# CliMA/OrthogonalSphericalShellGrids.jl

Measured on AMD Instinct MI355X. Metric: grid-cells/s metric precompute + zipper halo-fill GB/s, 1/10°×75z, higher is better.
Workload: dtype f64

## Files before the change

### orthogonalsphericalshellgrids.jl_amd/csrc/tpg_batch.hpp

```cpp
#pragma once
#include "tpg_math.hpp"

namespace tpgb {
using namespace tpgm;

#define TPG_UNROLL _Pragma("unroll")

template <int N> TPG_DEV double kc(double c)
{
#if defined(__HIP_DEVICE_COMPILE__)
    if (N == 1) asm("" : "+s"(c));
#endif
    return c;
}

template <int N> TPG_DEV void ksin_b(const double (&x)[N], const double (&y)[N], double (&out)[N])
{
    double z[N], r[N], v[N];
    TPG_UNROLL for (int e = 0; e < N; ++e) z[e] = x[e] * x[e];
    TPG_UNROLL for (int e = 0; e < N; ++e) r[e] = fmaD(z[e], kc<N>(1.58969099521155010221e-10), kc<N>(-2.50507602534068634195e-08));
    TPG_UNROLL for (int e = 0; e < N; ++e) r[e] = fmaD(z[e], r[e], kc<N>(2.75573137070700676789e-06));
    TPG_UNROLL for (int e = 0; e < N; ++e) r[e] = fmaD(z[e], r[e], kc<N>(-1.98412698298579493134e-04));
    TPG_UNROLL for (int e = 0; e < N; ++e) r[e] = fmaD(z[e], r[e], kc<N>(8.33333333332248946124e-03));
    TPG_UNROLL for (int e = 0; e < N; ++e) v[e] = z[e] * x[e];
// ... 8 lines not shown
    TPG_UNROLL for (int e = 0; e < N; ++e) r[e] = fmaD(z[e], r[e], kc<N>(-2.75573143513906633035e-07));
    TPG_UNROLL for (int e = 0; e < N; ++e) r[e] = fmaD(z[e], r[e], kc<N>(2.48015872894767294178e-05));
    TPG_UNROLL for (int e = 0; e < N; ++e) r[e] = fmaD(z[e], r[e], kc<N>(-1.38888888888741095749e-03));
    TPG_UNROLL for (int e = 0; e < N; ++e) r[e] = fmaD(z[e], r[e], kc<N>(4.16666666666666019037e-02));
    TPG_UNROLL for (int e = 0; e < N; ++e) r[e] = z[e] * r[e];
    TPG_UNROLL for (int e = 0; e < N; ++e) {
        double hz = 0.5 * z[e];
        double w = 1.0 - hz;
        out[e] = w + (((1.0 - w) - hz) + (z[e] * r[e] - x[e] * y[e]));
    }
}

template <int N> TPG_DEV void ksin0_b(const double (&x)[N], double (&out)[N])
{
    double z[N], r[N], v[N];
    TPG_UNROLL for (int e = 0; e < N; ++e) z[e] = x[e] * x[e];
    TPG_UNROLL for (int e = 0; e < N; ++e) r[e] = fmaD(z[e], kc<N>(1.58969099521155010221e-10), kc<N>(-2.50507602534068634195e-08));
    TPG_UNROLL for (int e = 0; e < N; ++e) r[e] = fmaD(z[e], r[e], kc<N>(2.75573137070700676789e-06));
    TPG_UNROLL for (int e = 0; e < N; ++e) r[e] = fmaD(z[e], r[e], kc<N>(-1.98412698298579493134e-04));
    TPG_UNROLL for (int e = 0; e < N; ++e) r[e] = fmaD(z[e], r[e], kc<N>(8.33333333332248946124e-03));
    TPG_UNROLL for (int e = 0; e < N; ++e) v[e] = z[e] * x[e];
    TPG_UNROLL for (int e = 0; e < N; ++e) {
        const double t = v[e] * r[e];
        out[e] = x[e] - (z[e] * -t - v[e] * kc<N>(-1.66666666666666324348e-01));
    }
}

template <int N> TPG_DEV bool sin_small_b(const double (&x)[N], double (&out)[N])
{
    bool rare = false;
    TPG_UNROLL for (int e = 0; e < N; ++e) rare |= !(absD(x[e]) <= kPio4Hi);
    ksin0_b<N>(x, out);
    return rare;
}

template <int N> TPG_DEV bool cos_b(const double (&a)[N], double (&out)[N])
{
    double fn[N], y0[N], y1[N], S[N], C[N];
    bool rare = false;
    TPG_UNROLL for (int e = 0; e < N; ++e) fn[e] = __builtin_rint(a[e] * kInvPio2);
    TPG_UNROLL for (int e = 0; e < N; ++e) {
        double r = a[e] - fn[e] * kPio2_1;
        double w = fn[e] * kPio2_1t;
        y0[e] = r - w;
        y1[e] = (r - y0[e]) - w;
        rare |= absD(y0[e]) < absD(a[e]) * 0x1p-15;
    }
    bool odd = false, even = false;
    TPG_UNROLL for (int e = 0; e < N; ++e) { const int n = (int)fn[e]; odd |= (n & 1) != 0; even |= (n & 1) == 0; }
    TPG_UNROLL for (int e = 0; e < N; ++e) { S[e] = 0.0; C[e] = 0.0; }
    if (__any(odd)) ksin_b<N>(y0, y1, S);
    if (__any(even)) kcos_b<N>(y0, y1, C);
    TPG_UNROLL for (int e = 0; e < N; ++e) {
        const int n = (int)fn[e];
        const double v = (n & 1) ? S[e] : C[e];
        const double nv = -v;
        out[e] = ((n + 1) & 2) ? nv : v;
    }
    return rare;
}

template <int N> TPG_DEV bool cos_lat_b(const double (&a)[N], double (&out)[N])
{
    double fn[N], y0[N], y1[N], S[N], C[N];
    bool rare = false;
    TPG_UNROLL for (int e = 0; e < N; ++e) fn[e] = __builtin_rint(a[e] * kInvPio2);
// ... 36 lines not shown
        num = b1 ? n1 : num; den = b1 ? d1 : den; h = b1 ? h1 : h; l = b1 ? l1 : l;
        num = b0 ? n0 : num; den = b0 ? d0 : den; h = b0 ? h0 : h; l = b0 ? l0 : l;
        hi[e] = h; lo[e] = l;
        double q = num / den;
        asm volatile("" : "+v"(q));
        t[e] = direct[e] ? ax : q;
    }
    {
        double z[N], w[N], s1[N], s2[N];
        TPG_UNROLL for (int e = 0; e < N; ++e) { z[e] = t[e] * t[e]; w[e] = z[e] * z[e]; }
        TPG_UNROLL for (int e = 0; e < N; ++e) { s1[e] = fmaD(w[e], 1.62858201153657823623e-02, 4.97687799461593236017e-02);
                                                 s2[e] = fmaD(w[e], -3.65315727442169155270e-02, -5.83357013379057348645e-02); }
        TPG_UNROLL for (int e = 0; e < N; ++e) { s1[e] = fmaD(w[e], s1[e], 6.66107313738753120669e-02);
                                                 s2[e] = fmaD(w[e], s2[e], -7.69187620504482999495e-02); }
        TPG_UNROLL for (int e = 0; e < N; ++e) { s1[e] = fmaD(w[e], s1[e], 9.09088713343650656196e-02);
                                                 s2[e] = fmaD(w[e], s2[e], -1.11111104054623557880e-01); }
        TPG_UNROLL for (int e = 0; e < N; ++e) { s1[e] = fmaD(w[e], s1[e], 1.42857142725034663711e-01);
                                                 s2[e] = fmaD(w[e], s2[e], -1.99999999998764832476e-01); }
        TPG_UNROLL for (int e = 0; e < N; ++e) { s1[e] = fmaD(w[e], s1[e], 3.33333333333329318027e-01);
                                                 s2[e] = w[e] * s2[e]; }
        TPG_UNROLL for (int e = 0; e < N; ++e) s[e] = z[e] * s1[e] + s2[e];
    }
    TPG_UNROLL for (int e = 0; e < N; ++e) {
        const double ts = t[e] * s[e];
        const double rd = t[e] - ts, rg = hi[e] - ((ts - lo[e]) - t[e]);
        const double r = direct[e] ? rd : rg;
        out[e] = csign(r, x[e]);
    }
}

struct AtanRow { double p, q, r, s, hi, lo; };
#define TPG_ATAN_ROWS_DOUBLES 30
#define TPG_ATAN_TABLE_DOUBLES 42
__device__ const unsigned kAtanLutWords[24] = {
    0x30303000u, 0x30303030u, 0x30303030u, 0x30303030u, 0x30303030u, 0x60606030u, 0x60606060u, 0x60606060u,
    0x60606060u, 0x60606060u, 0x60606060u, 0x90606060u, 0x90909090u, 0x90909090u, 0x90909090u, 0x90909090u,
    0x90909090u, 0x90909090u, 0x90909090u, 0x90909090u, 0xC0C0C0C0u, 0xC0C0C0C0u, 0xC0C0C0C0u, 0xC0C0C0C0u };
TPG_DEV void atan_table_init(double* tab, int tid)
{
    if (tid < 24) reinterpret_cast<unsigned*>(tab + TPG_ATAN_ROWS_DOUBLES)[tid] = kAtanLutWords[tid];
    const double rows[5][6] = {
        { 1.0, 0.0, 1.0, 0.0, 0.0, 0.0 },
        { 2.0, 1.0, 2.0, 1.0, 0x1.dac670561bb4fp-2, 0x1.a2b7f222f65e2p-56 },
        { 1.0, 1.0, 1.0, 1.0, 0x1.921fb54442d18p-1, 0x1.1a62633145c07p-55 },
        { 1.0, 1.5, 1.0, 1.5, 0x1.f730bd281f69bp-1, 0x1.007887af0cbbdp-56 },
        { 0.0, 1.0, 0.0, 1.0, kPio2Hi, kPio2Lo } };
    if (tid < TPG_ATAN_ROWS_DOUBLES) tab[tid] = rows[tid / 6][tid % 6];
}

template <int N, bool FINITE = false> TPG_DEV void atan_tab_b(const double (&x)[N], double (&out)[N], const double* tab)
{
    double t[N], hi[N], lo[N], s[N];
    TPG_UNROLL for (int e = 0; e < N; ++e) {
        const double ax = absD(x[e]);
        int u = (int)__builtin_amdgcn_ubfe((unsigned)__double2hiint(x[e]), 15u, 16u) - 0x7FB7;
        u = u < 0 ? 0 : (u > 80 ? 80 : u);
        const unsigned off = reinterpret_cast<const unsigned char*>(tab + TPG_ATAN_ROWS_DOUBLES)[u];
        const AtanRow row = *reinterpret_cast<const AtanRow*>(reinterpret_cast<const char*>(tab) + off);
        hi[e] = row.hi; lo[e] = row.lo;
        const double axn = (!FINITE && ax > 0x1p1000) ? 0x1p1000 : ax;
        const double num = row.p * axn - row.q;
        const double den = row.r + row.s * axn;
        double q = tpgm::div_nr(num, den);
        asm volatile("" : "+v"(q));
        t[e] = q;
    }
    {
        double z[N], w[N], s1[N], s2[N];
        TPG_UNROLL for (int e = 0; e < N; ++e) { z[e] = t[e] * t[e]; w[e] = z[e] * z[e]; }
        TPG_UNROLL for (int e = 0; e < N; ++e) { s1[e] = fmaD(w[e], 1.62858201153657823623e-02, 4.97687799461593236017e-02);
                                                 s2[e] = fmaD(w[e], -3.65315727442169155270e-02, -5.83357013379057348645e-02); }
        TPG_UNROLL for (int e = 0; e < N; ++e) { s1[e] = fmaD(w[e], s1[e], 6.66107313738753120669e-02);
                                                 s2[e] = fmaD(w[e], s2[e], -7.69187620504482999495e-02); }
        TPG_UNROLL for (int e = 0; e < N; ++e) { s1[e] = fmaD(w[e], s1[e], 9.09088713343650656196e-02);
                                                 s2[e] = fmaD(w[e], s2[e], -1.11111104054623557880e-01); }
        TPG_UNROLL for (int e = 0; e < N; ++e) { s1[e] = fmaD(w[e], s1[e], 1.42857142725034663711e-01);
                                                 s2[e] = fmaD(w[e], s2[e], -1.99999999998764832476e-01); }
        TPG_UNROLL for (int e = 0; e < N; ++e) { s1[e] = fmaD(w[e], s1[e], 3.33333333333329318027e-01);
                                                 s2[e] = w[e] * s2[e]; }
        TPG_UNROLL for (int e = 0; e < N; ++e) s[e] = z[e] * s1[e] + s2[e];
// ... 88 lines not shown
    double h[N], l[N], S[N], C[N];
    bool s1[N], c1[N], rare = false;
    TPG_UNROLL for (int e = 0; e < N; ++e) {
        const double r = absD(x[e]);
        rare |= !(r <= 90.0);
        s1[e] = r >= 45.0; c1[e] = r > 45.0;
        const double d = (s1[e] ? 90.0 : 0.0) - r;
        const double t = absD(d);
        const double hh = t * kDeg2Rad;
        l[e] = fmaD(t, kDeg2Rad, -hh) + t * kDeg2RadLo;
        h[e] = hh;
    }
    ksin_b<N>(h, l, S);
    kcos_b<N>(h, l, C);
    TPG_UNROLL for (int e = 0; e < N; ++e) {
        const double bs = s1[e] ? C[e] : S[e];
        sn[e] = csign(1.0, x[e]) * bs;
        cs[e] = c1[e] ? S[e] : C[e];
    }
    return rare;
}

TPG_DEV double fmod360_pos(double x)
{
    return x - __hiloint2double(!(x < 360.0) ? 0x40768000 : 0, 0);
}

TPG_DEV double fmod360_small(double x)
{
    const double ax = absD(x);
    return csign(ax - __hiloint2double(!(ax < 360.0) ? 0x40768000 : 0, 0), x);
}

}
```

### orthogonalsphericalshellgrids.jl_amd/csrc/tpg_grid.hip

```cpp
#include "tpg_common.hpp"
#include "tpg_math.hpp"
#include "tpg_batch.hpp"

using namespace tpgm;

namespace {

constexpr double kC180Pi = 180.0 / kPi;
constexpr double kC360Pi = 360.0 / kPi;

struct GridK {
    int Nx, Ny, Hx, Hy;
    int shift;
    int jstart, jend;
    int jm_lo, jm_hi;
    int sx, rows;
    int ft;
    double fplp90;
    double R;
    const double* ti;
    const double* tj;
    const double* ts;
};

// ... 162 lines not shown
}
__device__ __forceinline__ double tri_area(V3 a, V3 b, V3 c)
{
    double t = absD(dot3(a, cross3(b, c)));
    t /= 1 + dot3(a, b) + dot3(b, c) + dot3(a, c);
    return 2 * atanD(t);
}
__device__ __forceinline__ double quad_area(V3 a, V3 b, V3 c, V3 d)
{
    double A = tri_area(a, b, c);
    A += tri_area(a, b, d);
    A += tri_area(a, c, d);
    A += tri_area(b, c, d);
    return A / 2;
}

__device__ __forceinline__ double tri_tan_nr(V3 a, V3 b, V3 c)
{
    return div_nr(absD(dot3(a, cross3(b, c))), 1 + dot3(a, b) + dot3(b, c) + dot3(a, c));
}
__device__ __forceinline__ double tri_tan(V3 a, V3 b, V3 c)
{
    return absD(dot3(a, cross3(b, c))) / (1 + dot3(a, b) + dot3(b, c) + dot3(a, c));
}

template <typename T, bool NT = false>
__device__ __forceinline__ void put(const OutPtrs& o, int q, long long off, double v)
{
    T* p = static_cast<T*>(o.p[q]) + off;
    if (NT) __builtin_nontemporal_store((T)v, p); else *p = (T)v;
}

template <typename T, bool NT = false>
__device__ __forceinline__ void put32(const OutPtrs& o, int q, unsigned boff, double v)
{
    asm volatile("" : "+v"(boff));
    T* p = reinterpret_cast<T*>(static_cast<char*>(o.p[q]) + boff);
    if (NT) __builtin_nontemporal_store((T)v, p); else *p = (T)v;
}

template <typename T, bool NT>
__global__ __launch_bounds__(256) void k_cells(GridK g, OutPtrs o)
{
    const int nbx = (g.Nx + 255) / 256;
    int rb = blockIdx.x / nbx;
    int i = (blockIdx.x - rb * nbx) * 256 + threadIdx.x + 1;
    int j = g.jm_lo + rb;
    if (i > g.Nx) return;

    LP cc = coord(g, 0, 0, i, j), fc = coord(g, 1, 0, i, j), cf = coord(g, 0, 1, i, j), ff = coord(g, 1, 1, i, j);
    LP fc_e = coord(g, 1, 0, i + 1, j), fc_s = coord(g, 1, 0, i, j - 1);
    LP cc_w = coord(g, 0, 0, i - 1, j), cc_s = coord(g, 0, 0, i, j - 1), cc_sw = coord(g, 0, 0, i - 1, j - 1);
    LP ff_e = coord(g, 1, 1, i + 1, j), ff_n = coord(g, 1, 1, i, j + 1), ff_ne = coord(g, 1, 1, i + 1, j + 1);
    LP cf_w = coord(g, 0, 1, i - 1, j), cf_n = coord(g, 0, 1, i, j + 1);

    const double R = g.R;
    double dxcc = haversine(fc_e, fc, R);
    double dxfc = haversine(cc, cc_w, R);
    double dxcf = haversine(ff_e, ff, R);
    double dxff = haversine(cf, cf_w, R);
    double dycc = haversine(cf_n, cf, R);
    double dyfc = haversine(ff_n, ff, R);
    double dycf = haversine(cc, cc_s, R);
    double dyff = haversine(fc, fc_s, R);
    double azcc = quad_area(cartesian(ff), cartesian(ff_e), cartesian(ff_ne), cartesian(ff_n)) * (R * R);
    double azfc = dyfc * dxfc;
    double azcf = dycf * dxcf;
    double azff = quad_area(cartesian(cc_sw), cartesian(cc_s), cartesian(cc), cartesian(cc_w)) * (R * R);

    long long off = (long long)(i + g.Hx - 1) + (long long)g.sx * (j - g.jstart + g.Hy);
    put<T, NT>(o, TPG_LAMBDA_CC, off, cc.lam); put<T, NT>(o, TPG_LAMBDA_FC, off, fc.lam);
    put<T, NT>(o, TPG_LAMBDA_CF, off, cf.lam); put<T, NT>(o, TPG_LAMBDA_FF, off, ff.lam);
    put<T, NT>(o, TPG_PHI_CC, off, cc.phi); put<T, NT>(o, TPG_PHI_FC, off, fc.phi);
    put<T, NT>(o, TPG_PHI_CF, off, cf.phi); put<T, NT>(o, TPG_PHI_FF, off, ff.phi);
    put<T, NT>(o, TPG_DX_CC, off, dxcc); put<T, NT>(o, TPG_DX_FC, off, dxfc);
    put<T, NT>(o, TPG_DX_CF, off, dxcf); put<T, NT>(o, TPG_DX_FF, off, dxff);
    put<T, NT>(o, TPG_DY_CC, off, dycc); put<T, NT>(o, TPG_DY_CF, off, dycf);
    put<T, NT>(o, TPG_DY_FC, off, dyfc); put<T, NT>(o, TPG_DY_FF, off, dyff);
    put<T, NT>(o, TPG_AZ_CC, off, azcc); put<T, NT>(o, TPG_AZ_FC, off, azfc);
    put<T, NT>(o, TPG_AZ_CF, off, azcf); put<T, NT>(o, TPG_AZ_FF, off, azff);
}

struct Pt  { double lam, phi, a, ca; };
struct PtX { double lam, phi, a, ca, X, Y, Z; };
struct Nb  { double lam, a, ca; };
struct NbX { double lam, a, ca, X, Y, Z; };

__device__ __forceinline__ Pt make_pt(const GridK& g, int xl, int yl, int i, int j)
{
    LP p = coord(g, xl, yl, i, j);
    Pt r; r.lam = p.lam; r.phi = p.phi; r.a = p.phi * kDeg2Rad; r.ca = cosD(r.a);
    return r;
}
__device__ __forceinline__ PtX make_ptx(const GridK& g, int xl, int yl, int i, int j)
{
    LP p = coord(g, xl, yl, i, j);
    PtX r; r.lam = p.lam; r.phi = p.phi; r.a = p.phi * kDeg2Rad; r.ca = cosD(r.a);
    double sl, cl, sp, cp;
    sincosd(p.lam, sl, cl);
    sincosd(p.phi, sp, cp);
    r.X = cl * cp; r.Y = sl * cp; r.Z = sp;
    return r;
}
__device__ __forceinline__ Nb nb_of(const Pt& p) { return Nb{ p.lam, p.a, p.ca }; }
__device__ __forceinline__ Nb nb_of(const PtX& p) { return Nb{ p.lam, p.a, p.ca }; }
__device__ __forceinline__ NbX nbx_of(const PtX& p) { return NbX{ p.lam, p.a, p.ca, p.X, p.Y, p.Z }; }
__device__ __forceinline__ V3 v3_of(const PtX& p) { return V3{ p.X, p.Y, p.Z }; }
__device__ __forceinline__ V3 v3_of(const NbX& p) { return V3{ p.X, p.Y, p.Z }; }

template <int DIR> __device__ __forceinline__ double shf(double v)
{
    return DIR > 0 ? __shfl_down(v, 1, 64) : __shfl_up(v, 1, 64);
}
template <int DIR> __device__ __forceinline__ Nb shf_nb(const Pt& p)
{
    return Nb{ shf<DIR>(p.lam), shf<DIR>(p.a), shf<DIR>(p.ca) };
}
template <int DIR> __device__ __forceinline__ NbX shf_nbx(const PtX& p)
// ... 58 lines not shown
    tpgb::sincosd_b<4>(ang, sn, cs);
    s.X[0] = cs[0] * cs[1]; s.Y[0] = sn[0] * cs[1]; s.Z[0] = sn[1];
    s.X[1] = cs[2] * cs[3]; s.Y[1] = sn[2] * cs[3]; s.Z[1] = sn[3];
}

template <int R>
__device__ __forceinline__ void points_pair(const GridK& g, const LaneConst& lc, const RowTab& rt, Step4& s, const double* atab,
                                            double (*L)[R][64], int p, int lane)
{
    const bool face = lane >= 32;
    const double aslO = face ? lc.aslF : lc.aslC, aclO = face ? lc.aclF : lc.aclC;
    {
        const double x[2] = { aslO * rt.chC, aslO * rt.chF };
        const double y[2] = { aclO * rt.shC, aclO * rt.shF };
        double q[2], rr[2], at1[2], at2[2], phi[2], a[2], ca[2];
        bool zerox = false;
#pragma unroll
        for (int m = 0; m < 2; ++m) { q[m] = div_nr(y[m], x[m]); zerox |= x[m] == 0.0; rr[m] = sqrt_nr<true>(y[m] * y[m] + x[m] * x[m]);    }
        tpgb::atan_tab_b<2, true>(q, at1, atab);
        tpgb::atan_tab_b<2, true>(rr, at2, atab);
        if (zerox) {
#pragma unroll
            for (int m = 0; m < 2; ++m)
                if (x[m] == 0.0) {
                    const double qq = y[m] / x[m];
                    at1[m] = (qq != qq) ? qq : csign(kPio2Hi, qq);
                }
        }
#pragma unroll
        for (int m = 0; m < 2; ++m) { phi[m] = 90.0 - kC360Pi * at2[m]; a[m] = phi[m] * kDeg2Rad; }
        if (tpgb::cos_lat_b<2>(a, ca)) { ca[0] = cosD(a[0]); ca[1] = cosD(a[1]); }
        double lat[1] = { face ? phi[1] : phi[0] }, sp[1], cp[1];
        if (tpgb::sincosd_lat_b<1>(lat, sp, cp)) tpgb::sincosd_b<1>(lat, sp, cp);
        const int k0 = face ? 0 : 1;
        L[3 * k0 + 0][p][lane] = at1[0]; L[3 * k0 + 1][p][lane] = phi[0]; L[3 * k0 + 2][p][lane] = ca[0];
        L[3 * k0 + 6][p][lane] = at1[1]; L[3 * k0 + 7][p][lane] = phi[1]; L[3 * k0 + 8][p][lane] = ca[1];
        L[14 - 2 * k0][p][lane] = sp[0]; L[15 - 2 * k0][p][lane] = cp[0];
    }
    __builtin_amdgcn_fence(__ATOMIC_RELEASE, "wavefront");
    __builtin_amdgcn_wave_barrier();
    __builtin_amdgcn_fence(__ATOMIC_ACQUIRE, "wavefront");
    const int srcF = face ? lane : (lane == 0 ? 63 : 64 - lane), srcC = face ? 63 - lane : lane;
    const int sgn = (int)0x80000000;
    int sgJc = __double2hiint(rt.shC) & sgn, sgJf = __double2hiint(rt.shF) & sgn;
    int sgF = (__double2hiint(lc.aslF) ^ __double2hiint(lc.aclF)) & sgn, sgC = (__double2hiint(lc.aslC) ^ __double2hiint(lc.aclC)) & sgn;
    asm volatile("" : "+v"(sgF), "+v"(sgC), "+s"(sgJc), "+s"(sgJf));
    double at1[4], sp[2], cp[2];
#pragma unroll
    for (int k = 0; k < 4; ++k) {
        const int src = (k == 0 || k == 2) ? srcF : srcC;
        at1[k] = L[3 * k + 0][p][src];
        s.phi[k] = L[3 * k + 1][p][src];
        s.ca[k] = L[3 * k + 2][p][src];
    }
    sp[0] = L[12][p][srcC]; cp[0] = L[13][p][srcC];
    sp[1] = L[14][p][srcF]; cp[1] = L[15][p][srcF];
    __builtin_amdgcn_fence(__ATOMIC_RELEASE, "wavefront");
    __builtin_amdgcn_wave_barrier();
    __builtin_amdgcn_fence(__ATOMIC_ACQUIRE, "wavefront");
    const bool lsmall = (__double2hiint(g.fplp90) & 0x7fffffff) < 0x40666000;
    const double cJc = __hiloint2double(__double2hiint(-kC180Pi) ^ sgJc, __double2loint(-kC180Pi));
    const double cJf = __hiloint2double(__double2hiint(-kC180Pi) ^ sgJf, __double2loint(-kC180Pi));
    double l[4];
#pragma unroll
    for (int k = 0; k < 4; ++k) {
        const double m = ((k < 2) ? cJc : cJf) * absD(at1[k]);
        l[k] = __hiloint2double(__double2hiint(m) ^ ((k == 0 || k == 2) ? sgF : sgC), __double2loint(m));
        l[k] += lc.hemi;
        l[k] += g.fplp90;
        s.a[k] = s.phi[k] * kDeg2Rad;
    }
    if (lsmall) {
#pragma unroll
        for (int k = 0; k < 4; ++k) s.lam[k] = tpgb::fmod360_pos(l[k] + 360.0);
    } else {
#pragma unroll
        for (int k = 0; k < 4; ++k) s.lam[k] = tpgb::fmod360_pos(tpgb::fmod360_small(l[k]) + 360.0);
    }
    double lon[2] = { s.lam[1], s.lam[2] }, sl[2], cl[2];
    tpgb::sincosd_b<2, true>(lon, sl, cl);
    s.X[0] = cl[0] * cp[0]; s.Y[0] = sl[0] * cp[0]; s.Z[0] = sp[0];
    s.X[1] = cl[1] * cp[1]; s.Y[1] = sl[1] * cp[1]; s.Z[1] = sp[1];
}

__device__ __forceinline__ int wrap_col(int v, int Nx)
{
    if (v < 1) v += Nx;
    if (v > Nx) v -= Nx;
    if (v < 1 || v > Nx) { v = (v - 1) % Nx; v = (v < 0 ? v + Nx : v) + 1; }
    return v;
}

__device__ __noinline__ void points_general(const GridK& g, int i, int jc, int jf, Step4& s)
{
    Pt fc = make_pt(g, 1, 0, i, jc), cf = make_pt(g, 0, 1, i, jf);
    PtX cc = make_ptx(g, 0, 0, i, jc), ff = make_ptx(g, 1, 1, i, jf);
    s.lam[0] = fc.lam; s.phi[0] = fc.phi; s.a[0] = fc.a; s.ca[0] = fc.ca;
    s.lam[1] = cc.lam; s.phi[1] = cc.phi; s.a[1] = cc.a; s.ca[1] = cc.ca;
    s.lam[2] = ff.lam; s.phi[2] = ff.phi; s.a[2] = ff.a; s.ca[2] = ff.ca;
    s.lam[3] = cf.lam; s.phi[3] = cf.phi; s.a[3] = cf.a; s.ca[3] = cf.ca;
    s.X[0] = cc.X; s.Y[0] = cc.Y; s.Z[0] = cc.Z;
    s.X[1] = ff.X; s.Y[1] = ff.Y; s.Z[1] = ff.Z;
}

template <int R> struct TileLds { double v[18][R][64]; };
enum { L_FC = 0, L_CC = 3, L_FF = 9, L_CF = 15 };

template <int N>
__device__ __forceinline__ void hav_batch(const Nb (&X)[N], const Nb (&Y)[N], double Rad, double (&d)[N])
{
    double hp[N], hl[N], s1[N], s2[N], hh[N], rt[N], rm[N], as[N];
    bool zero = false;
#pragma unroll
    for (int e = 0; e < N; ++e) {
        double dp = Y[e].a - X[e].a;
        hp[e] = dp / 2; hl[e] = (Y[e].lam - X[e].lam) * (kDeg2Rad * 0.5);
    }
    if (tpgb::sin_small_b<N>(hp, s1)) {
#pragma unroll
        for (int e = 0; e < N; ++e) s1[e] = sinD(hp[e]);
    }
    if (tpgb::sin_small_b<N>(hl, s2)) {
#pragma unroll
        for (int e = 0; e < N; ++e) s2[e] = sinD(hl[e]);
    }
#pragma unroll
    for (int e = 0; e < N; ++e) {
        double h = s1[e] * s1[e] + X[e].ca * Y[e].ca * (s2[e] * s2[e]);
        hh[e] = h;
        zero |= h == 0.0;
        rt[e] = sqrt_nr<true>(h);
    }
    if (zero) {
#pragma unroll
        for (int e = 0; e < N; ++e) rt[e] = sqrt_nr(hh[e]);
    }
#pragma unroll
    for (int e = 0; e < N; ++e) {
        rm[e] = __builtin_fmin(rt[e], 1.0);
    }
    if (tpgb::asin_small_b<N>(rm, as)) {
#pragma unroll
        for (int e = 0; e < N; ++e) as[e] = asinD(!(rt[e] >= 1.0) ? rt[e] : 1.0);
    }
#pragma unroll
    for (int e = 0; e < N; ++e) d[e] = (2 * Rad) * as[e];
}

#ifndef TPG_CELLS_PROBE
#define TPG_CELLS_PROBE 0
#endif
#if TPG_CELLS_PROBE == 2 || TPG_CELLS_PROBE == 3
#define TPG_EMIT(A, OFF, V) (fold ^= (unsigned long long)__double_as_longlong(V) + (A), fold_off = (OFF), folded = true)
#else
#define TPG_EMIT(A, OFF, V) put32<T, NT>(o, A, OFF, V)
#endif

__device__ __forceinline__ int tile_of_block(int b, int tiles, bool grouped)
{
    const int base = b & ~63;
    if (grouped && base + 64 <= tiles) return base + (b & 7) * 8 + ((b >> 3) & 7);
    return b;
}

template <typename T, bool NT, int R>
__global__ __launch_bounds__(64 * R, 4) void k_cells_tile(GridK g, OutPtrs o, int tiles_x, int tiles, int grouped)
{
    __shared__ __attribute__((aligned(16))) double atabs[R][TPG_ATAN_TABLE_DOUBLES];
    __shared__ TileLds<R> lds;
    const int lane = threadIdx.x & 63;
    const int p = __builtin_amdgcn_readfirstlane(threadIdx.x >> 6);
    double* atab = atabs[p];
    tpgb::atan_table_init(atab, lane);
    __builtin_amdgcn_fence(__ATOMIC_RELEASE, "wavefront");
    __builtin_amdgcn_wave_barrier();
    __builtin_amdgcn_fence(__ATOMIC_ACQUIRE, "wavefront");
    const int tiles_y = tiles / tiles_x;
    const int hl = lane & 31;
    const double Rad = g.R;
    const bool fast_grid = absD(g.fplp90) <= 360.0;
#if TPG_CELLS_PROBE == 2 || TPG_CELLS_PROBE == 3
    unsigned long long fold = 0; unsigned fold_off = 0; bool folded = false;
#endif

    const int t = tile_of_block((int)blockIdx.x, tiles, grouped != 0);
    const int ty = tiles_y - 1 - t / tiles_x, tx = t % tiles_x;
    const int s0 = g.jm_lo - 1 + ty * (R - 1);
    const int s = s0 + p;
    const int i = wrap_col(lane >= 32 ? g.shift - 30 * tx - 30 + hl : g.shift + 30 * tx + hl, g.Nx);
    const bool col_emit = hl >= 1 && hl <= 30 && 30 * tx + (lane >= 32 ? 30 - hl : hl - 1) < g.Nx / 2;
    const bool active_row = s <= g.jm_hi;
    const unsigned col = (unsigned)(i + g.Hx - 1);
    auto rowoff = [&](int j) -> unsigned { return (col + (unsigned)g.sx * (unsigned)(j - g.jstart + g.Hy)) * (unsigned)sizeof(T); };
    LaneConst lc;
#if TPG_CELLS_PROBE == 3
    const RowTab rt = RowTab{ 0.5 + 1e-3 * (s & 7), 1.1, 0.6, 1.2 };
    lc.aslF = 0.31 + 0.01 * hl; lc.aclF = 0.72 + 1e-3 * (i & 1); lc.aslC = 0.33 + 0.01 * hl; lc.aclC = 0.74;
#else
    const RowTab rt = load_rowtab(g, s, s + 1);
    lc.aslF = g.ti[0 * g.Nx + i - 1]; lc.aclF = g.ti[1 * g.Nx + i - 1];
    lc.aslC = g.ti[2 * g.Nx + i - 1]; lc.aclC = g.ti[3 * g.Nx + i - 1];
#endif

    Step4 q;
    if (active_row) {
        const bool fast = s >= 1 && s < g.Ny && fast_grid;
        if (fast) {
            int i0 = i - g.shift; if (i0 < 1) i0 += g.Nx;
            lc.hemi = (i0 <= g.Nx / 2) ? -90.0 : 90.0;
#if TPG_CELLS_PROBE == 1
            const double pv = (lc.aslF + lc.aclC) * rt.shC + (double)(tx + lane);
#pragma unroll
            for (int k = 0; k < 4; ++k) { q.lam[k] = pv; q.phi[k] = pv; q.a[k] = pv; q.ca[k] = pv; }
            q.X[0] = q.Y[0] = q.Z[0] = q.X[1] = q.Y[1] = q.Z[1] = pv;
#else
            points_pair<R>(g, lc, rt, q, atab, lds.v, p, lane);
#endif
        } else {
            Step4 tmp; GridK gc = g; points_general(gc, i, s, s + 1, tmp); q = tmp;
        }
        if (col_emit) {
            if (p >= 1 && s >= g.jm_lo) {
                unsigned off = rowoff(s);
                TPG_EMIT(TPG_LAMBDA_FC, off, q.lam[0]); TPG_EMIT(TPG_PHI_FC, off, q.phi[0]);
                TPG_EMIT(TPG_LAMBDA_CC, off, q.lam[1]); TPG_EMIT(TPG_PHI_CC, off, q.phi[1]);
            }
            if ((p >= 1 || ty == 0) && s + 1 >= g.jm_lo && s + 1 <= g.jm_hi) {
                unsigned off1 = rowoff(s + 1);
                TPG_EMIT(TPG_LAMBDA_FF, off1, q.lam[2]); TPG_EMIT(TPG_PHI_FF, off1, q.phi[2]);
                TPG_EMIT(TPG_LAMBDA_CF, off1, q.lam[3]); TPG_EMIT(TPG_PHI_CF, off1, q.phi[3]);
            }
        }
        double (*L)[R][64] = lds.v;
        L[L_FC + 0][p][lane] = q.lam[0]; L[L_FC + 1][p][lane] = q.a[0]; L[L_FC + 2][p][lane] = q.ca[0];
        L[L_CC + 0][p][lane] = q.lam[1]; L[L_CC + 1][p][lane] = q.a[1]; L[L_CC + 2][p][lane] = q.ca[1];
        L[L_CC + 3][p][lane] = q.X[0];   L[L_CC + 4][p][lane] = q.Y[0]; L[L_CC + 5][p][lane] = q.Z[0];
        L[L_FF + 0][p][lane] = q.lam[2]; L[L_FF + 1][p][lane] = q.a[2]; L[L_FF + 2][p][lane] = q.ca[2];
        L[L_FF + 3][p][lane] = q.X[1];   L[L_FF + 4][p][lane] = q.Y[1]; L[L_FF + 5][p][lane] = q.Z[1];
        L[L_CF + 0][p][lane] = q.lam[3]; L[L_CF + 1][p][lane] = q.a[3]; L[L_CF + 2][p][lane] = q.ca[3];
    }
    __syncthreads();
    if (p == 0) {
        if (col_emit) {
            double (*L)[R][64] = lds.v;
            int r = 1;
#pragma unroll 1
            for (; r + 1 < R && s0 + r + 1 <= g.jm_hi; r += 2) {
                const int sa = s0 + r, sb = sa + 1;
                double dd2[2];
#if TPG_CELLS_PROBE == 1
                dd2[0] = dd2[1] = L[L_FC + 0][r][lane];
#else
                Nb X[2] = { Nb{ L[L_FC + 0][r][lane], L[L_FC + 1][r][lane], L[L_FC + 2][r][lane] },
                            Nb{ L[L_FC + 0][r + 1][lane], L[L_FC + 1][r + 1][lane], L[L_FC + 2][r + 1][lane] } };
                Nb Y[2] = { Nb{ L[L_FC + 0][r - 1][lane], L[L_FC + 1][r - 1][lane], L[L_FC + 2][r - 1][lane] }, X[0] };
                hav_batch<2>(X, Y, Rad, dd2);
#endif
                if (sa >= g.jm_lo) TPG_EMIT(TPG_DY_FF, rowoff(sa), dd2[0]);
                if (sb >= g.jm_lo) TPG_EMIT(TPG_DY_FF, rowoff(sb), dd2[1]);
            }
            if (r < R && s0 + r <= g.jm_hi) {
                const int sa = s0 + r;
                double dd1[1];
#if TPG_CELLS_PROBE == 1
                dd1[0] = L[L_FC + 0][r][lane];
#else
                Nb X[1] = { Nb{ L[L_FC + 0][r][lane], L[L_FC + 1][r][lane], L[L_FC + 2][r][lane] } };
                Nb Y[1] = { Nb{ L[L_FC + 0][r - 1][lane], L[L_FC + 1][r - 1][lane], L[L_FC + 2][r - 1][lane] } };
                hav_batch<1>(X, Y, Rad, dd1);
#endif
                if (sa >= g.jm_lo) TPG_EMIT(TPG_DY_FF, rowoff(sa), dd1[0]);
            }
        }
    } else if (active_row && s >= g.jm_lo) {
        if (col_emit) {
        double (*L)[R][64] = lds.v;
        const int pm = p - 1, le = lane + 1, lw = lane - 1;
        const unsigned off = rowoff(s);
        double d[8];
#if TPG_CELLS_PROBE == 1
        {
            const double pv = q.lam[0] + L[L_FC + 0][pm][le];
            TPG_EMIT(TPG_AZ_CC, off, pv); TPG_EMIT(TPG_AZ_FF, off, pv);
#pragma unroll
            for (int k = 0; k < 8; ++k) d[k] = pv;
        }
#else
#pragma unroll
        for (int k = 0; k < 2; ++k) {
            V3 a, b, c, dd;
            if (k == 0) {
                a = V3{ L[L_FF + 3][pm][lane], L[L_FF + 4][pm][lane], L[L_FF + 5][pm][lane] };
                b = V3{ L[L_FF + 3][pm][le], L[L_FF + 4][pm][le], L[L_FF + 5][pm][le] };
                c = V3{ L[L_FF + 3][p][le], L[L_FF + 4][p][le], L[L_FF + 5][p][le] };
                dd = V3{ q.X[1], q.Y[1], q.Z[1] };
            } else {
                a = V3{ L[L_CC + 3][pm][lw], L[L_CC + 4][pm][lw], L[L_CC + 5][pm][lw] };
                b = V3{ L[L_CC + 3][pm][lane], L[L_CC + 4][pm][lane], L[L_CC + 5][pm][lane] };
                c = V3{ q.X[0], q.Y[0], q.Z[0] };
                dd = V3{ L[L_CC + 3][p][lw], L[L_CC + 4][p][lw], L[L_CC + 5][p][lw] };
            }
            double tt[4], at[4];
            tt[0] = tri_tan_nr(a, b, c); tt[1] = tri_tan_nr(a, b, dd);
            tt[2] = tri_tan_nr(a, c, dd); tt[3] = tri_tan_nr(b, c, dd);
            if (__any(tpgb::atan_small_b<4>(tt, at))) {
                tt[0] = tri_tan(a, b, c); tt[1] = tri_tan(a, b, dd); tt[2] = tri_tan(a, c, dd); tt[3] = tri_tan(b, c, dd);
                tpgb::atan_b<4>(tt, at);
            }
            double A = at[0];
            A += at[1];
            A += at[2];
// ... 120 lines not shown

size_t table_doubles(const tpg_params* p) { return 4 * (size_t)p->Nx + 4 * (size_t)p->Ny + 5 * (size_t)(p->Hy + 1); }

int check_params(const tpg_params* p)
{
    if (!p) { tpg::set_error("null params"); return TPG_ERR_INVALID_ARGUMENT; }
    int rc = tpg::check_geom(p->Nx, p->Ny, p->Nz, p->Hx, p->Hy, p->Hz, p->ft);
    if (rc) return rc;
    if (p->jstart < 1 || p->jend > p->Ny || p->jend < p->jstart) {
        tpg::set_error("latitude band %d:%d outside 1:%d", p->jstart, p->jend, p->Ny);
        return TPG_ERR_BAD_PARTITION;
    }
    if (p->reserved & ~TPG_BUILD_TABLES_VALID) {
        tpg::set_error("tpg_params.reserved: unknown flag bits 0x%x", p->reserved & ~TPG_BUILD_TABLES_VALID);
        return TPG_ERR_INVALID_ARGUMENT;
    }
    if (!(p->radius > 0) || !(p->north_poles_latitude < 90) || !(p->southernmost_latitude < 90)) {
        tpg::set_error("invalid radius / latitudes");
        return TPG_ERR_INVALID_ARGUMENT;
    }
    return TPG_OK;
}

template <typename T>
int launch_build(const GridK& g, const OutPtrs& o, const HaloRegions& h, hipStream_t s)
{
    dim3 grid1(((g.Nx + 255) / 256) * (g.jm_hi - g.jm_lo + 1));
    const tpg::Config& cfg = tpg::config();
    const bool nt = cfg.build_nt;
    int rc = TPG_OK;
    constexpr int R = 8;
    const int nrows = g.jm_hi - g.jm_lo + 1;
    const int tiles_y = (nrows + (R - 1) - 1) / (R - 1);
    const bool offsets32 = (unsigned long long)g.sx * (unsigned long long)(g.jend - g.jstart + 1 + 2 * g.Hy) * sizeof(T) < (1ull << 32);
    const bool south_in_band = g.jstart - g.Hy <= 1;
    const bool tile = cfg.cells_variant != 0 && tiles_y <= 65535 && offsets32;
    if (tile) {
        const int tiles_x = (g.Nx / 2 + 29) / 30;
        const int tiles = tiles_x * tiles_y;
        if (nt) hipLaunchKernelGGL((k_cells_tile<T, true, R>), dim3((unsigned)tiles), dim3(64 * R), 0, s, g, o, tiles_x, tiles, cfg.cells_order);
        else    hipLaunchKernelGGL((k_cells_tile<T, false, R>), dim3((unsigned)tiles), dim3(64 * R), 0, s, g, o, tiles_x, tiles, cfg.cells_order);
    }
    else if (nt) hipLaunchKernelGGL((k_cells<T, true>), grid1, dim3(256), 0, s, g, o);
    else         hipLaunchKernelGGL((k_cells<T, false>), grid1, dim3(256), 0, s, g, o);
    if ((rc = tpg::launch_status("k_cells"))) return rc;
    HaloRegions hm = h;
    hm.merged_south = (south_in_band && g.Ny > 2 * g.Hy + 2) ? 1 : 0;
    if (hm.merged_south) hm.nC = (h.nsouth + 1) * g.sx;
    int nh = hm.nA + hm.nB + hm.nC + hm.nD;
    if (nh > 0) {
        hipLaunchKernelGGL(k_halos<T>, dim3((nh + 255) / 256, TPG_NUM_ARRAYS), dim3(256), 0, s, g, o, hm);
        if ((rc = tpg::launch_status("k_halos"))) return rc;
    }
    if (south_in_band && !hm.merged_south) {
        hipLaunchKernelGGL(k_south<T>, dim3((g.sx + 255) / 256, g.Hy + 1), dim3(256), 0, s, g, o);
        if ((rc = tpg::launch_status("k_south"))) return rc;
    }
    return TPG_OK;
}

}

extern "C" {

size_t tpg_build_grid_workspace_bytes(const tpg_params* p)
{
    if (!p || p->Nx < 1 || p->Ny < 1 || p->Hy < 0) return 0;
    return (table_doubles(p) * sizeof(double) + 255) & ~(size_t)255;
}

int tpg_build_grid(const tpg_params* p, void* const out[TPG_NUM_ARRAYS], void* workspace,
                   size_t workspace_bytes, void* stream)
{
    int rc = check_params(p);
// ... 46 lines not shown
```

### orthogonalsphericalshellgrids.jl_amd/csrc/tpg_math.hpp

```cpp
#pragma once
#include <hip/hip_runtime.h>
#include <stdint.h>

namespace tpgm {

#define TPG_DEV __device__ __forceinline__

constexpr double kPi       = 0x1.921fb54442d18p+1;
constexpr double kDeg2Rad  = 0x1.1df46a2529d39p-6;
constexpr double kDeg2RadLo = 0x1.5c1d8becdd291p-62;
constexpr double kInvPio2  = 0x1.45f306dc9c883p-1;
constexpr double kPio2_1   = 0x1.921fb54400000p+0;
constexpr double kPio2_1t  = 0x1.0b4611a626331p-34;
constexpr double kPio2_2   = 0x1.0b4611a600000p-34;
constexpr double kPio2_2t  = 0x1.3198a2e037073p-69;
constexpr double kPio2_3   = 0x1.3198a2e000000p-69;
constexpr double kPio2_3t  = 0x1.b839a252049c1p-104;
constexpr double kPio2Hi   = 0x1.921fb54442d18p+0;
constexpr double kPio2Lo   = 0x1.1a62633145c07p-54;
constexpr double kPio4Hi   = 0x1.921fb54442d18p-1;
constexpr double kLn2Hi    = 0x1.62e42fefa39efp-1;
constexpr double kLn2Lo    = 0x1.abc9e3b39803fp-56;

TPG_DEV uint64_t bits(double x) { return (uint64_t)__double_as_longlong(x); }
// ... 347 lines not shown
{
    int e = expo(a.hi) - 1023;
    double m = from_bits((bits(a.hi) & 0x000fffffffffffffull) | 0x3ff0000000000000ull);
    if (m > 0x1.6a09e667f3bcdp+0) { m *= 0.5; e += 1; }
    double u = (m - 1.0) / (m + 1.0), u2 = u * u;
    double ser = u * (2.0 + u2 * (2.0 / 3.0 + u2 * (2.0 / 5.0 + u2 * (2.0 / 7.0 + u2 * (2.0 / 9.0
                 + u2 * (2.0 / 11.0 + u2 * (2.0 / 13.0 + u2 * (2.0 / 15.0 + u2 * (2.0 / 17.0 + u2 * (2.0 / 19.0))))))))));
    dd y = two_sum((double)e * kLn2Hi, ser);
    for (int it = 0; it < 1; ++it) {
        dd ey = dd_exp(dd_neg(y));
        dd c = dd_sub(dd_mul(a, ey), dd{ 1.0, 0.0 });
        y = dd_add(y, c);
    }
    return y;
}
TPG_DEV double asinhD(double x)
{
    double ax = absD(x);
    if (ax == 0.0 || x != x) return x;
    dd s = dd_sqrt(dd_add(two_prod(ax, ax), dd{ 1.0, 0.0 }));
    dd l = dd_log(dd_add(dd{ ax, 0.0 }, s));
    return csign(l.hi + l.lo, x);
}
TPG_DEV void sinh_cosh(double x, double& sh, double& ch)
{
    double ax = absD(x);
    dd e = dd_exp(dd{ ax, 0.0 });
    dd ie = dd_div(dd{ 1.0, 0.0 }, e);
    dd s = dd_sub(e, ie), c = dd_add(e, ie);
    sh = csign(0.5 * (s.hi + s.lo), x);
    ch = 0.5 * (c.hi + c.lo);
}

}
```

Measured before the change: 12.91 billion.

## Micro-optimize tile kernel: magic-number division, packed LDS, table copy, cheaper wrap

```diff
diff --git a/orthogonalsphericalshellgrids.jl_amd/csrc/tpg_batch.hpp b/orthogonalsphericalshellgrids.jl_amd/csrc/tpg_batch.hpp
--- a/orthogonalsphericalshellgrids.jl_amd/csrc/tpg_batch.hpp
+++ b/orthogonalsphericalshellgrids.jl_amd/csrc/tpg_batch.hpp
@@ -64,6 +64,14 @@
     TPG_UNROLL for (int e = 0; e < N; ++e) rare |= !(absD(x[e]) <= kPio4Hi);
     ksin0_b<N>(x, out);
     return rare;
+}
+
+template <int N> TPG_DEV bool sin_small_sum_b(const double (&x)[N], double (&out)[N])
+{
+    double m = absD(x[0]);
+    TPG_UNROLL for (int e = 1; e < N; ++e) m += absD(x[e]);
+    ksin0_b<N>(x, out);
+    return !(m <= kPio4Hi);
 }
 
 template <int N> TPG_DEV bool cos_b(const double (&a)[N], double (&out)[N])
@@ -166,20 +174,21 @@
 struct AtanRow { double p, q, r, s, hi, lo; };
 #define TPG_ATAN_ROWS_DOUBLES 30
 #define TPG_ATAN_TABLE_DOUBLES 42
-__device__ const unsigned kAtanLutWords[24] = {
-    0x30303000u, 0x30303030u, 0x30303030u, 0x30303030u, 0x30303030u, 0x60606030u, 0x60606060u, 0x60606060u,
-    0x60606060u, 0x60606060u, 0x60606060u, 0x90606060u, 0x90909090u, 0x90909090u, 0x90909090u, 0x90909090u,
-    0x90909090u, 0x90909090u, 0x90909090u, 0x90909090u, 0xC0C0C0C0u, 0xC0C0C0C0u, 0xC0C0C0C0u, 0xC0C0C0C0u };
+struct AtanTableImage { double rows[TPG_ATAN_ROWS_DOUBLES]; unsigned lut[24]; };
+static_assert(sizeof(AtanTableImage) == TPG_ATAN_TABLE_DOUBLES * sizeof(double), "atan table image");
+__device__ const AtanTableImage kAtanTable = {
+    { 1.0, 0.0, 1.0, 0.0, 0.0, 0.0,
+      2.0, 1.0, 2.0, 1.0, 0x1.dac670561bb4fp-2, 0x1.a2b7f222f65e2p-56,
+      1.0, 1.0, 1.0, 1.0, 0x1.921fb54442d18p-1, 0x1.1a62633145c07p-55,
+      1.0, 1.5, 1.0, 1.5, 0x1.f730bd281f69bp-1, 0x1.007887af0cbbdp-56,
+      0.0, 1.0, 0.0, 1.0, kPio2Hi, kPio2Lo },
+    { 0x30303000u, 0x30303030u, 0x30303030u, 0x30303030u, 0x30303030u, 0x60606030u, 0x60606060u, 0x60606060u,
+      0x60606060u, 0x60606060u, 0x60606060u, 0x90606060u, 0x90909090u, 0x90909090u, 0x90909090u, 0x90909090u,
+      0x90909090u, 0x90909090u, 0x90909090u, 0x90909090u, 0xC0C0C0C0u, 0xC0C0C0C0u, 0xC0C0C0C0u, 0xC0C0C0C0u } };
 TPG_DEV void atan_table_init(double* tab, int tid)
 {
-    if (tid < 24) reinterpret_cast<unsigned*>(tab + TPG_ATAN_ROWS_DOUBLES)[tid] = kAtanLutWords[tid];
-    const double rows[5][6] = {
-        { 1.0, 0.0, 1.0, 0.0, 0.0, 0.0 },
-        { 2.0, 1.0, 2.0, 1.0, 0x1.dac670561bb4fp-2, 0x1.a2b7f222f65e2p-56 },
-        { 1.0, 1.0, 1.0, 1.0, 0x1.921fb54442d18p-1, 0x1.1a62633145c07p-55 },
-        { 1.0, 1.5, 1.0, 1.5, 0x1.f730bd281f69bp-1, 0x1.007887af0cbbdp-56 },
-        { 0.0, 1.0, 0.0, 1.0, kPio2Hi, kPio2Lo } };
-    if (tid < TPG_ATAN_ROWS_DOUBLES) tab[tid] = rows[tid / 6][tid % 6];
+    if ((unsigned)tid < (unsigned)TPG_ATAN_TABLE_DOUBLES)
+        reinterpret_cast<unsigned long long*>(tab)[tid] = reinterpret_cast<const unsigned long long*>(&kAtanTable)[tid];
 }
 
 template <int N, bool FINITE = false> TPG_DEV void atan_tab_b(const double (&x)[N], double (&out)[N], const double* tab)
@@ -334,4 +343,38 @@
     return csign(ax - __hiloint2double(!(ax < 360.0) ? 0x40768000 : 0, 0), x);
 }
 
-}
+struct Nb { double lam, a, ca; };
+
+template <int N>
+TPG_DEV void hav_batch(const Nb (&X)[N], const Nb (&Y)[N], double Rad, double (&d)[N])
+{
+    double hp[N], hl[N], s1[N], s2[N], hh[N], rt[N], rm[N], as[N];
+    bool zero = false;
+    TPG_UNROLL for (int e = 0; e < N; ++e) {
+        double dp = Y[e].a - X[e].a;
+        hp[e] = dp / 2; hl[e] = (Y[e].lam - X[e].lam) * (kDeg2Rad * 0.5);
+    }
+    if (sin_small_sum_b<N>(hp, s1)) {
+        TPG_UNROLL for (int e = 0; e < N; ++e) s1[e] = sinD(hp[e]);
+    }
+    if (sin_small_sum_b<N>(hl, s2)) {
+        TPG_UNROLL for (int e = 0; e < N; ++e) s2[e] = sinD(hl[e]);
+    }
+    TPG_UNROLL for (int e = 0; e < N; ++e) {
+        double h = s1[e] * s1[e] + X[e].ca * Y[e].ca * (s2[e] * s2[e]);
+        hh[e] = h;
+        zero |= h == 0.0;
+        rt[e] = sqrt_nr<true>(h);
+        rm[e] = __builtin_fmin(rt[e], 1.0);
+    }
+    if (zero) {
+        asm volatile("");
+        TPG_UNROLL for (int e = 0; e < N; ++e) { rt[e] = sqrt_nr(hh[e]); rm[e] = __builtin_fmin(rt[e], 1.0); }
+    }
+    if (asin_small_b<N>(rm, as)) {
+        TPG_UNROLL for (int e = 0; e < N; ++e) as[e] = asinD(!(rt[e] >= 1.0) ? rt[e] : 1.0);
+    }
+    TPG_UNROLL for (int e = 0; e < N; ++e) d[e] = (2 * Rad) * as[e];
+}
+
+}
diff --git a/orthogonalsphericalshellgrids.jl_amd/csrc/tpg_grid.hip b/orthogonalsphericalshellgrids.jl_amd/csrc/tpg_grid.hip
--- a/orthogonalsphericalshellgrids.jl_amd/csrc/tpg_grid.hip
+++ b/orthogonalsphericalshellgrids.jl_amd/csrc/tpg_grid.hip
@@ -218,7 +218,7 @@
 }
 
 template <typename T, bool NT = false>
-__device__ __forceinline__ void put32(const OutPtrs& o, int q, unsigned boff, double v)
+__device__ __forceinline__ void put32(const OutPtrs& o, int q, unsigned& boff, double v)
 {
     asm volatile("" : "+v"(boff));
     T* p = reinterpret_cast<T*>(static_cast<char*>(o.p[q]) + boff);
@@ -269,7 +269,7 @@
 
 struct Pt  { double lam, phi, a, ca; };
 struct PtX { double lam, phi, a, ca, X, Y, Z; };
-struct Nb  { double lam, a, ca; };
+using tpgb::Nb;
 struct NbX { double lam, a, ca, X, Y, Z; };
 
 __device__ __forceinline__ Pt make_pt(const GridK& g, int xl, int yl, int i, int j)
@@ -394,10 +394,9 @@
         if (tpgb::cos_lat_b<2>(a, ca)) { ca[0] = cosD(a[0]); ca[1] = cosD(a[1]); }
         double lat[1] = { face ? phi[1] : phi[0] }, sp[1], cp[1];
         if (tpgb::sincosd_lat_b<1>(lat, sp, cp)) tpgb::sincosd_b<1>(lat, sp, cp);
-        const int k0 = face ? 0 : 1;
-        L[3 * k0 + 0][p][lane] = at1[0]; L[3 * k0 + 1][p][lane] = phi[0]; L[3 * k0 + 2][p][lane] = ca[0];
-        L[3 * k0 + 6][p][lane] = at1[1]; L[3 * k0 + 7][p][lane] = phi[1]; L[3 * k0 + 8][p][lane] = ca[1];
-        L[14 - 2 * k0][p][lane] = sp[0]; L[15 - 2 * k0][p][lane] = cp[0];
+        L[0][p][lane] = at1[0]; L[1][p][lane] = phi[0]; L[2][p][lane] = ca[0];
+        L[3][p][lane] = at1[1]; L[4][p][lane] = phi[1]; L[5][p][lane] = ca[1];
+        L[6][p][lane] = sp[0];  L[7][p][lane] = cp[0];
     }
     __builtin_amdgcn_fence(__ATOMIC_RELEASE, "wavefront");
     __builtin_amdgcn_wave_barrier();
@@ -410,17 +409,19 @@
     double at1[4], sp[2], cp[2];
 #pragma unroll
     for (int k = 0; k < 4; ++k) {
-        const int src = (k == 0 || k == 2) ? srcF : srcC;
-        at1[k] = L[3 * k + 0][p][src];
-        s.phi[k] = L[3 * k + 1][p][src];
-        s.ca[k] = L[3 * k + 2][p][src];
-    }
-    sp[0] = L[12][p][srcC]; cp[0] = L[13][p][srcC];
-    sp[1] = L[14][p][srcF]; cp[1] = L[15][p][srcF];
+        const int src = (k == 0 || k == 2) ? srcF : srcC, c = k >> 1;
+        at1[k] = L[3 * c + 0][p][src];
+        s.phi[k] = L[3 * c + 1][p][src];
+        s.ca[k] = L[3 * c + 2][p][src];
+    }
+    sp[0] = L[6][p][srcC]; cp[0] = L[7][p][srcC];
+    sp[1] = L[6][p][srcF]; cp[1] = L[7][p][srcF];
     __builtin_amdgcn_fence(__ATOMIC_RELEASE, "wavefront");
     __builtin_amdgcn_wave_barrier();
     __builtin_amdgcn_fence(__ATOMIC_ACQUIRE, "wavefront");
-    const bool lsmall = (__double2hiint(g.fplp90) & 0x7fffffff) < 0x40666000;
+    int fph = __double2hiint(g.fplp90) & 0x7fffffff;
+    asm("" : "+s"(fph));
+    const bool lsmall = fph < 0x40666000;
     const double cJc = __hiloint2double(__double2hiint(-kC180Pi) ^ sgJc, __double2loint(-kC180Pi));
     const double cJf = __hiloint2double(__double2hiint(-kC180Pi) ^ sgJf, __double2loint(-kC180Pi));
     double l[4];
@@ -445,13 +446,6 @@
     s.X[1] = cl[1] * cp[1]; s.Y[1] = sl[1] * cp[1]; s.Z[1] = sp[1];
 }
 
-__device__ __forceinline__ int wrap_col(int v, int Nx)
-{
-    if (v < 1) v += Nx;
-    if (v > Nx) v -= Nx;
-    if (v < 1 || v > Nx) { v = (v - 1) % Nx; v = (v < 0 ? v + Nx : v) + 1; }
-    return v;
-}
 
 __device__ __noinline__ void points_general(const GridK& g, int i, int jc, int jf, Step4& s)
 {
@@ -468,46 +462,7 @@
 template <int R> struct TileLds { double v[18][R][64]; };
 enum { L_FC = 0, L_CC = 3, L_FF = 9, L_CF = 15 };
 
-template <int N>
-__device__ __forceinline__ void hav_batch(const Nb (&X)[N], const Nb (&Y)[N], double Rad, double (&d)[N])
-{
-    double hp[N], hl[N], s1[N], s2[N], hh[N], rt[N], rm[N], as[N];
-    bool zero = false;
-#pragma unroll
-    for (int e = 0; e < N; ++e) {
-        double dp = Y[e].a - X[e].a;
-        hp[e] = dp / 2; hl[e] = (Y[e].lam - X[e].lam) * (kDeg2Rad * 0.5);
-    }
-    if (tpgb::sin_small_b<N>(hp, s1)) {
-#pragma unroll
-        for (int e = 0; e < N; ++e) s1[e] = sinD(hp[e]);
-    }
-    if (tpgb::sin_small_b<N>(hl, s2)) {
-#pragma unroll
-        for (int e = 0; e < N; ++e) s2[e] = sinD(hl[e]);
-    }
-#pragma unroll
-    for (int e = 0; e < N; ++e) {
-        double h = s1[e] * s1[e] + X[e].ca * Y[e].ca * (s2[e] * s2[e]);
-        hh[e] = h;
-        zero |= h == 0.0;
-        rt[e] = sqrt_nr<true>(h);
-    }
-    if (zero) {
-#pragma unroll
-        for (int e = 0; e < N; ++e) rt[e] = sqrt_nr(hh[e]);
-    }
-#pragma unroll
-    for (int e = 0; e < N; ++e) {
-        rm[e] = __builtin_fmin(rt[e], 1.0);
-    }
-    if (tpgb::asin_small_b<N>(rm, as)) {
-#pragma unroll
-        for (int e = 0; e < N; ++e) as[e] = asinD(!(rt[e] >= 1.0) ? rt[e] : 1.0);
-    }
-#pragma unroll
-    for (int e = 0; e < N; ++e) d[e] = (2 * Rad) * as[e];
-}
+using tpgb::hav_batch;
 
 #ifndef TPG_CELLS_PROBE
 #define TPG_CELLS_PROBE 0
@@ -525,8 +480,15 @@
     return b;
 }
 
+struct TileGeom { int tiles_x, tiles_y, tiles, grouped; UDiv by_tiles_x; };
+
+__device__ __forceinline__ double ldtab32(const double* base, unsigned boff)
+{
+    return *reinterpret_cast<const double*>(reinterpret_cast<const char*>(base) + boff);
+}
+
 template <typename T, bool NT, int R>
-__global__ __launch_bounds__(64 * R, 4) void k_cells_tile(GridK g, OutPtrs o, int tiles_x, int tiles, int grouped)
+__global__ __launch_bounds__(64 * R, 4) void k_cells_tile(GridK g, OutPtrs o, TileGeom tg)
 {
     __shared__ __attribute__((aligned(16))) double atabs[R][TPG_ATAN_TABLE_DOUBLES];
     __shared__ TileLds<R> lds;
@@ -537,7 +499,7 @@
     __builtin_amdgcn_fence(__ATOMIC_RELEASE, "wavefront");
     __builtin_amdgcn_wave_barrier();
     __builtin_amdgcn_fence(__ATOMIC_ACQUIRE, "wavefront");
-    const int tiles_y = tiles / tiles_x;
+    const int tiles_x = tg.tiles_x, tiles_y = tg.tiles_y;
     const int hl = lane & 31;
     const double Rad = g.R;
     const bool fast_grid = absD(g.fplp90) <= 360.0;
@@ -545,8 +507,9 @@
     unsigned long long fold = 0; unsigned fold_off = 0; bool folded = false;
 #endif
 
-    const int t = tile_of_block((int)blockIdx.x, tiles, grouped != 0);
-    const int ty = tiles_y - 1 - t / tiles_x, tx = t % tiles_x;
+    const int t = tile_of_block((int)blockIdx.x, tg.tiles, tg.grouped != 0);
+    const int trow = (int)udiv((unsigned)t, tg.by_tiles_x);
+    const int ty = tiles_y - 1 - trow, tx = t - trow * tiles_x;
     const int s0 = g.jm_lo - 1 + ty * (R - 1);
     const int s = s0 + p;
     const int i = wrap_col(lane >= 32 ? g.shift - 30 * tx - 30 + hl : g.shift + 30 * tx + hl, g.Nx);
@@ -560,8 +523,9 @@
     lc.aslF = 0.31 + 0.01 * hl; lc.aclF = 0.72 + 1e-3 * (i & 1); lc.aslC = 0.33 + 0.01 * hl; lc.aclC = 0.74;
 #else
     const RowTab rt = load_rowtab(g, s, s + 1);
-    lc.aslF = g.ti[0 * g.Nx + i - 1]; lc.aclF = g.ti[1 * g.Nx + i - 1];
-    lc.aslC = g.ti[2 * g.Nx + i - 1]; lc.aclC = g.ti[3 * g.Nx + i - 1];
+    const unsigned tioff = (unsigned)(i - 1) * (unsigned)sizeof(double);
+    lc.aslF = ldtab32(g.ti + 0 * (size_t)g.Nx, tioff); lc.aclF = ldtab32(g.ti + 1 * (size_t)g.Nx, tioff);
+    lc.aslC = ldtab32(g.ti + 2 * (size_t)g.Nx, tioff); lc.aclC = ldtab32(g.ti + 3 * (size_t)g.Nx, tioff);
 #endif
 
     Step4 q;
@@ -618,8 +582,9 @@
                 Nb Y[2] = { Nb{ L[L_FC + 0][r - 1][lane], L[L_FC + 1][r - 1][lane], L[L_FC + 2][r - 1][lane] }, X[0] };
                 hav_batch<2>(X, Y, Rad, dd2);
 #endif
-                if (sa >= g.jm_lo) TPG_EMIT(TPG_DY_FF, rowoff(sa), dd2[0]);
-                if (sb >= g.jm_lo) TPG_EMIT(TPG_DY_FF, rowoff(sb), dd2[1]);
+                unsigned offa = rowoff(sa), offb = rowoff(sb);
+                if (sa >= g.jm_lo) TPG_EMIT(TPG_DY_FF, offa, dd2[0]);
+                if (sb >= g.jm_lo) TPG_EMIT(TPG_DY_FF, offb, dd2[1]);
             }
             if (r < R && s0 + r <= g.jm_hi) {
                 const int sa = s0 + r;
@@ -631,14 +596,15 @@
                 Nb Y[1] = { Nb{ L[L_FC + 0][r - 1][lane], L[L_FC + 1][r - 1][lane], L[L_FC + 2][r - 1][lane] } };
                 hav_batch<1>(X, Y, Rad, dd1);
 #endif
-                if (sa >= g.jm_lo) TPG_EMIT(TPG_DY_FF, rowoff(sa), dd1[0]);
+                unsigned offa = rowoff(sa);
+                if (sa >= g.jm_lo) TPG_EMIT(TPG_DY_FF, offa, dd1[0]);
             }
         }
     } else if (active_row && s >= g.jm_lo) {
         if (col_emit) {
         double (*L)[R][64] = lds.v;
         const int pm = p - 1, le = lane + 1, lw = lane - 1;
-        const unsigned off = rowoff(s);
+        unsigned off = rowoff(s);
         double d[8];
 #if TPG_CELLS_PROBE == 1
         {
@@ -825,14 +791,16 @@
     constexpr int R = 8;
     const int nrows = g.jm_hi - g.jm_lo + 1;
     const int tiles_y = (nrows + (R - 1) - 1) / (R - 1);
-    const bool offsets32 = (unsigned long long)g.sx * (unsigned long long)(g.jend - g.jstart + 1 + 2 * g.Hy) * sizeof(T) < (1ull << 32);
+    const bool offsets32 = (unsigned long long)g.sx * (unsigned long long)(g.jend - g.jstart + 1 + 2 * g.Hy) * sizeof(T) < (1ull << 32)
+                           && (unsigned long long)g.Nx * sizeof(double) < (1ull << 32);
     const bool south_in_band = g.jstart - g.Hy <= 1;
     const bool tile = cfg.cells_variant != 0 && tiles_y <= 65535 && offsets32;
     if (tile) {
         const int tiles_x = (g.Nx / 2 + 29) / 30;
         const int tiles = tiles_x * tiles_y;
-        if (nt) hipLaunchKernelGGL((k_cells_tile<T, true, R>), dim3((unsigned)tiles), dim3(64 * R), 0, s, g, o, tiles_x, tiles, cfg.cells_order);
-        else    hipLaunchKernelGGL((k_cells_tile<T, false, R>), dim3((unsigned)tiles), dim3(64 * R), 0, s, g, o, tiles_x, tiles, cfg.cells_order);
+        const TileGeom tg = { tiles_x, tiles_y, tiles, cfg.cells_order, udiv_of((unsigned)tiles_x) };
+        if (nt) hipLaunchKernelGGL((k_cells_tile<T, true, R>), dim3((unsigned)tiles), dim3(64 * R), 0, s, g, o, tg);
+        else    hipLaunchKernelGGL((k_cells_tile<T, false, R>), dim3((unsigned)tiles), dim3(64 * R), 0, s, g, o, tg);
     }
     else if (nt) hipLaunchKernelGGL((k_cells<T, true>), grid1, dim3(256), 0, s, g, o);
     else         hipLaunchKernelGGL((k_cells<T, false>), grid1, dim3(256), 0, s, g, o);
diff --git a/orthogonalsphericalshellgrids.jl_amd/csrc/tpg_math.hpp b/orthogonalsphericalshellgrids.jl_amd/csrc/tpg_math.hpp
--- a/orthogonalsphericalshellgrids.jl_amd/csrc/tpg_math.hpp
+++ b/orthogonalsphericalshellgrids.jl_amd/csrc/tpg_math.hpp
@@ -403,4 +403,37 @@
     ch = 0.5 * (c.hi + c.lo);
 }
 
-}
+struct UDiv { unsigned mul; int sh1, sh2; };
+inline UDiv udiv_of(unsigned d)
+{
+    int l = 0;
+    while ((1ull << l) < d) ++l;
+    UDiv u;
+    u.mul = (unsigned)(((1ull << 32) * ((1ull << l) - d)) / d + 1);
+    u.sh1 = l < 1 ? l : 1;
+    u.sh2 = l > 1 ? l - 1 : 0;
+    return u;
+}
+TPG_DEV unsigned udiv(unsigned n, const UDiv& u)
+{
+    const unsigned t = (unsigned)(((unsigned long long)n * u.mul) >> 32);
+    return (t + ((n - t) >> u.sh1)) >> u.sh2;
+}
+
+constexpr int kWrapNear = 64;
+TPG_DEV int wrap_col_far(int v, int Nx)
+{
+    if (v < 1) v += Nx;
+    if (v > Nx) v -= Nx;
+    if (v < 1 || v > Nx) { v = (v - 1) % Nx; v = (v < 0 ? v + Nx : v) + 1; }
+    return v;
+}
+TPG_DEV int wrap_col(int v, int Nx)
+{
+    if (Nx < kWrapNear) return wrap_col_far(v, Nx);
+    if (v < 1) v += Nx;
+    if (v > Nx) v -= Nx;
+    return v;
+}
+
+}
```

New measurement: 13.04 billion (median of 3 runs). Within noise of the previous version (+1.0%).
